# Project-MONAI/MONAI

Hardware: AMD Instinct MI355X
Metric: voxels/s sliding-window 3D seg (512^3 vol, 96^3 win, ov 0.5) at 1/8 GPU (higher is better)
Workload: dtype f32; 1 GPU; BasicUNet 5-class seed 1, 512^3 CT phantom in HBM, 96^3 win ov 0.5 gaussian, sw_batch 4 (engine: <= 64 windows per launch); parallelism=1 GPU

## Files before the change

### monai_amd/csrc/kernels/conv3d_wino_h2.h

```cpp
#pragma once
#include "common.h"
#include "conv3d_h2.h"

namespace mh {

constexpr int HWG_BY = 4, HWG_BX = 16;
constexpr int HWG_RY = HWG_BY + 2, HWG_RX = HWG_BX + 2;
constexpr int HWG_NP = HWG_RY * HWG_RX;
constexpr int HWG_PB = 144;
constexpr int HWG_DB = (HWG_NP + 1) * HWG_PB;
constexpr int HWG_ZB = 32 * 1024;
constexpr int HWG_OPS = 24;
constexpr int HWG_CIN = 32, HWG_CN = 32;
constexpr int HWG_WAVES = 8;
constexpr unsigned HWG_DROP = 0x80000000u;

__device__ __forceinline__ void hw_split4(const f32x4 v, u32x2& hi, u32x2& lo) {
    _Float16 h_[4], l_[4];
#pragma unroll
    for (int i = 0; i < 4; ++i) {
        h_[i] = (_Float16)v[i];
        float r = v[i] - (float)h_[i];
        MH_OPAQUE(r);
        l_[i] = (_Float16)r;
    }
    const f16x2 h01 = {h_[0], h_[1]}, h23 = {h_[2], h_[3]}, l01 = {l_[0], l_[1]}, l23 = {l_[2], l_[3]};
    hi = u32x2{__builtin_bit_cast(unsigned, h01), __builtin_bit_cast(unsigned, h23)};
    lo = u32x2{__builtin_bit_cast(unsigned, l01), __builtin_bit_cast(unsigned, l23)};
}

__device__ __forceinline__ f32x4 hw_fma4(const f32x4 a, const float s, const f32x4 c) { return __builtin_elementwise_fma(a, f32x4{s, s, s, s}, c); }
__device__ __forceinline__ void hw_split4p(const f32x4 v, const float m1, u32x2& hi, u32x2& lo) {
#ifdef MH_SIMT_EMULATOR
    f16x2 h01, l01, h23, l23;
    h2_split_pair(v[0], v[1], m1, h01, l01);
    h2_split_pair(v[2], v[3], m1, h23, l23);
    hi = u32x2{__builtin_bit_cast(unsigned, h01), __builtin_bit_cast(unsigned, h23)};
    lo = u32x2{__builtin_bit_cast(unsigned, l01), __builtin_bit_cast(unsigned, l23)};
#else
    unsigned h0, h1, l0, l1;
    asm("v_cvt_pk_f16_f32 %0, %1, %2" : "=v"(h0) : "v"(v[0]), "v"(v[1]));
    asm("v_cvt_pk_f16_f32 %0, %1, %2" : "=v"(h1) : "v"(v[2]), "v"(v[3]));
    asm("v_fma_mixlo_f16 %0, %1, %2, %3 op_sel_hi:[1,0,0]" : "=v"(l0) : "v"(h0), "v"(m1), "v"(v[0]));
    asm("v_fma_mixlo_f16 %0, %1, %2, %3 op_sel_hi:[1,0,0]" : "=v"(l1) : "v"(h1), "v"(m1), "v"(v[2]));
    asm("v_fma_mixhi_f16 %0, %1, %2, %3 op_sel:[1,0,0] op_sel_hi:[1,0,0]" : "+v"(l0) : "v"(h0), "v"(m1), "v"(v[1]));
    asm("v_fma_mixhi_f16 %0, %1, %2, %3 op_sel:[1,0,0] op_sel_hi:[1,0,0]" : "+v"(l1) : "v"(h1), "v"(m1), "v"(v[3]));
    hi = u32x2{h0, h1};
    lo = u32x2{l0, l1};
#endif
}
__device__ __forceinline__ float hw_xchg32(const float x, const int hi) {
#ifdef MH_SIMT_EMULATOR
    (void)hi;
    return __shfl_xor(x, 32);
#else
    const auto r = __builtin_amdgcn_permlane32_swap(__builtin_bit_cast(unsigned, x), __builtin_bit_cast(unsigned, x), false, false);
    return __builtin_bit_cast(float, hi ? r[0] : r[1]);
#endif
}
#ifdef MH_SIMT_EMULATOR
#define MH_HW_KEEP_BRANCH ((void)0)
#else
#define MH_HW_KEEP_BRANCH asm volatile("" ::: "memory")
#endif

template <bool STATS, bool ACC = false, bool POOL = false>
__global__ void __launch_bounds__(512)
conv3d_k3_h2w_kernel(Tensor in, const uint4* __restrict__ wp, const float* __restrict__ wtail, const float* __restrict__ bias, Tensor out,
                     float* __restrict__ stats, int bxn, int byn, int zchunk, unsigned nblk, float* __restrict__ pmax, float* __restrict__ pmin,
                     long long pool_n_stride) {
    __shared__ __attribute__((aligned(16))) char smem[3 * HWG_DB + 2 * HWG_ZB];
    __shared__ unsigned bound_s[4];
    char* const ds = smem;
    char* const zs_ = smem + 3 * HWG_DB;
    const int tid = threadIdx.x, lane = tid & 63;
    const int wave = __builtin_amdgcn_readfirstlane(tid >> 6);
    const int wi = wave & 3, jp = wave >> 2;
    const int Cout = out.C, D = out.D, H = out.H, W = out.W;
    const long long HW = (long long)H * W, DHW = (long long)D * HW;

    const unsigned ncg = (unsigned)(Cout / HWG_CN);
    unsigned lid = xcd_remap(blockIdx.x, gridDim.x);
    const int cg = (int)(lid % ncg);
    lid /= ncg;
    const unsigned b = lid % nblk;
    const int n = (int)(lid / nblk);
    const int x0 = (int)(b % bxn) * HWG_BX, y0 = (int)((b / bxn) % byn) * HWG_BY;
    const int zs = (int)(b / (bxn * byn)) * zchunk, ze = min(zs + zchunk, D);
    const int p_first = max(zs - 1, 0), p_last = min(ze, D - 1);

    unsigned soff;
    int loff[2];
    {
        const int pr = min(lane, 53);
        const int ly = pr / 9;
        int lx = 2 * (pr - 9 * ly);
        const int gy = y0 + ly - 1;
        int gx = x0 + lx - 1;
        if (gx < 0) { gx += 1; lx += 1; }
        if (gx + 1 >= W) { gx -= 1; lx -= 1; }
        const bool ok = lane < 54 && gy >= 0 && gy < H;
        soff = ok ? 4u * (unsigned)(gy * W + gx) : 0u;
        loff[0] = (ok ? ly * HWG_RX + lx : HWG_NP) * HWG_PB;
        loff[1] = (ok ? ly * HWG_RX + lx + 1 : HWG_NP) * HWG_PB;
    }
    for (int i = tid; i < (3 * HWG_DB + 2 * HWG_ZB) / 16; i += 512) reinterpret_cast<uint4*>(smem)[i] = make_uint4(0u, 0u, 0u, 0u);
    f32x4 nra, nrb, nrs;
    {
        unsigned mb = 0u;
        if (lane < HWG_CIN) {
            const float4 a = *reinterpret_cast<const float4*>(in.nrm + (long long)n * in.nrm_n_stride + 4LL * lane);
            const unsigned bb = abs_bits(a.w);
            mb = bb == 0u ? 0x7fc00000u : bb;
        }
        mb = wave_umax(mb);
        if (tid == 0) bound_s[0] = mb;
    }
    __syncthreads();
    int e_in = 0;
    bool poisoned = false;
    {
        const unsigned mb = bound_s[0];
        poisoned = mb >= 0x7f800000u;
        e_in = poisoned ? 0 : min(max(13 - ((int)(mb >> 23) - 126), -100), 100);
        const float p_ = __uint_as_float((unsigned)(e_in + 127) << 23);
#pragma unroll
        for (int i = 0; i < 4; ++i) {
            const float4 a = *reinterpret_cast<const float4*>(in.nrm + (long long)n * in.nrm_n_stride + 4LL * (4 * wave + i));
            nra[i] = a.x * p_; nrb[i] = a.y * p_; nrs[i] = a.z;
        }
    }
    f32x4 nrk;
#pragma unroll
    for (int i = 0; i < 4; ++i) nrk[i] = nrs[i] <= 1.0f ? __builtin_inff() : -__builtin_inff();
    const auto xrs = __builtin_amdgcn_make_buffer_rsrc(const_cast<float*>(in.data + (long long)n * in.n_stride + (long long)(4 * wave) * DHW), 0, 0x7fffffff, 0x00020000);
    const unsigned hw4 = (unsigned)(HW * 4);
    unsigned voff = soff + (unsigned)p_first * hw4;
    const unsigned cso1 = (unsigned)(DHW * 4), cso2 = 2u * cso1, cso3 = 3u * cso1;
    f32x2 xin[4];
#define MH_HW_LDX                                                                                     \
    {                                                                                                 \
        xin[0] = __builtin_bit_cast(f32x2, __builtin_amdgcn_raw_buffer_load_b64(xrs, voff, 0u, 0));   \
        xin[1] = __builtin_bit_cast(f32x2, __builtin_amdgcn_raw_buffer_load_b64(xrs, voff, cso1, 0)); \
        xin[2] = __builtin_bit_cast(f32x2, __builtin_amdgcn_raw_buffer_load_b64(xrs, voff, cso2, 0)); \
        xin[3] = __builtin_bit_cast(f32x2, __builtin_amdgcn_raw_buffer_load_b64(xrs, voff, cso3, 0)); \
    }
#define MH_HW_CONV(DBO)                                                                               \
    {                                                                                                 \
        char* const db_ = ds + (DBO) + 16 * wave;                                                     \
        _Pragma("unroll") for (int j = 0; j < 2; ++j) {                                               \
            f32x4 y_;                                                                                 \
            const f32x4 t_ = __builtin_elementwise_fma(f32x4{xin[0][j], xin[1][j], xin[2][j], xin[3][j]}, nra, nrb), u_ = t_ * nrs; \
            _Pragma("unroll") for (int i = 0; i < 4; ++i) y_[i] = __builtin_amdgcn_fmed3f(t_[i], u_[i], nrk[i]);       \
            *reinterpret_cast<f32x4*>(db_ + loff[j]) = y_;                                            \
        }                                                                                             \
    }
    int staged = p_first;
#define MH_HW_ADV { voff += staged < p_last ? hw4 : 0u; staged += 1; }

    u32x4 wu[HWG_OPS];
    {
        const u32x4* wg = reinterpret_cast<const u32x4*>(wp) + ((long long)(cg * 8 + wave) * HWG_OPS) * 64 + lane;
#pragma unroll
        for (int r = 0; r < HWG_OPS; ++r) wu[r] = wg[r * 64];
    }
#define MH_HW_U(SL, T, CB, PC) __builtin_bit_cast(f16x8, wu[(((SL) * 3 + (T)) * 2 + (CB)) * 2 + (PC)])

    const int rho = lane & 15, kg = lane >> 4;
    const int tty = (rho >= 4 && rho < 12) ? 1 : 0, ttx = rho < 4 ? rho : rho < 12 ? rho - 4 : rho - 8;
    const int ra = wi == 0 ? 0 : wi == 2 ? 2 : 1, rb = wi == 0 ? 2 : wi == 1 ? 2 : wi == 2 ? 1 : 3;
    const float sgn = wi == 1 ? 1.0f : -1.0f;
    const float fsg = jp ? -1.0f : 1.0f;
    const float m1 = h2_minus_one();
    const int ab0 = ((2 * tty + ra) * HWG_RX + 2 * ttx + jp) * HWG_PB + kg * 16;
    const int ab1 = ((2 * tty + rb) * HWG_RX + 2 * ttx + jp) * HWG_PB + kg * 16;

    f32x4 acc[3][2][2];
#pragma unroll
    for (int s = 0; s < 3; ++s)
#pragma unroll
        for (int j = 0; j < 2; ++j)
#pragma unroll
            for (int c = 0; c < 2; ++c) acc[s][j][c] = f32x4{0.0f, 0.0f, 0.0f, 0.0f};

    const int fcb = wave >> 2, frp = (wave >> 1) & 1, fh = wave & 1;
    const int il = 32 * fh + (lane & 31), fa = lane >> 5;
    const int g4 = il >> 4;
    const int fty = (g4 == 1 || g4 == 2) ? 1 : 0, ftx = (g4 >= 2 ? 4 : 0) + 2 * frp;
    const int co_l = fcb * 16 + (il & 15), co = cg * HWG_CN + co_l;
    const float bco = bias ? bias[co] : 0.0f;
    const float fs2 = fa ? -1.0f : 1.0f;
    const int zwr = wave * 4096 + lane * 16;
    const int zrd = fa * 4096 + fcb * 2048 + il * 16 + frp * 8;
    float inv_a, inv_b;
    {
        const int t_ = -((int)((__float_as_uint(wtail[1]) >> 23) & 0xffu) - 127) - e_in;
        const int t1_ = t_ / 2, t2_ = t_ - t1_;
        inv_a = poisoned ? __uint_as_float(0x7fc00000u) : __uint_as_float((unsigned)(t1_ + 127) << 23);
        inv_b = __uint_as_float((unsigned)(t2_ + 127) << 23);
    }
    const auto orsrc = __builtin_amdgcn_make_buffer_rsrc(out.data + (long long)n * out.n_stride + (long long)(cg * HWG_CN) * DHW, 0, (int)(HWG_CN * DHW * 4), 0x00020000);
    const unsigned ooff = 4u * (unsigned)((long long)co_l * DHW + (long long)(y0 + 2 * fty + fa) * W + x0 + 2 * ftx);
    float pivot = 0.0f;
    bool have_c = false;
    f32x4 s1 = {0.0f, 0.0f, 0.0f, 0.0f}, s2 = s1;
    const long long PHW = (long long)(H / 2) * (W / 2), PDHW = (long long)(D / 2) * PHW;
    const auto prs = __builtin_amdgcn_make_buffer_rsrc(POOL ? (fa ? pmin : pmax) + (long long)n * pool_n_stride + (long long)(cg * HWG_CN) * PDHW : out.data, 0, POOL ? (int)(HWG_CN * PDHW * 4) : 0, 0x00020000);
    const unsigned poff = 4u * (unsigned)((long long)co_l * PDHW + (long long)((y0 >> 1) + fty) * (W / 2) + (x0 >> 1) + ftx);
    const float pk_ = fa ? -__builtin_inff() : __builtin_inff();
    f32x2 hm = {0.0f, 0.0f};
    f32x4 pv = {0.0f, 0.0f, 0.0f, 0.0f};

    u32x4 ah[2], al[2];
#define MH_HW_XFORM(DBO)                                                                              \
    {                                                                                                 \
        const char* const db_ = ds + (DBO);                                                           \
        _Pragma("unroll") for (int h = 0; h < 2; ++h) {                                               \
            f32x4 r_[3];                                                                              \
            _Pragma("unroll") for (int bq = 0; bq < 3; ++bq) {                                        \
                const f32x4 u_ = *reinterpret_cast<const f32x4*>(db_ + ab0 + bq * HWG_PB + h * 64);   \
                const f32x4 v_ = *reinterpret_cast<const f32x4*>(db_ + ab1 + bq * HWG_PB + h * 64);   \
                r_[bq] = hw_fma4(v_, sgn, u_);                                                        \
            }                                                                                         \
            const f32x4 e_ = hw_fma4(r_[2], m1, r_[0]);                                               \
            f32x4 f_;                                                                                 \
            if (jp) { f_ = hw_fma4(r_[0], m1, r_[1]); MH_HW_KEEP_BRANCH; } else f_ = r_[1] + r_[2];   \
            u32x2 hh_, ll_;                                                                           \
            hw_split4p(e_, m1, hh_, ll_); ah[0][2 * h] = hh_[0]; ah[0][2 * h + 1] = hh_[1]; al[0][2 * h] = ll_[0]; al[0][2 * h + 1] = ll_[1]; \
            hw_split4p(f_, m1, hh_, ll_); ah[1][2 * h] = hh_[0]; ah[1][2 * h + 1] = hh_[1]; al[1][2 * h] = ll_[0]; al[1][2 * h + 1] = ll_[1]; \
        }                                                                                             \
    }
#define MH_HW_MM(S, SL, CB, A, B, FRESH)                                                              \
    acc[S][SL][CB] = __builtin_amdgcn_mfma_f32_16x16x32_f16(__builtin_bit_cast(f16x8, A), B, (FRESH) ? f32x4{0.0f, 0.0f, 0.0f, 0.0f} : acc[S][SL][CB], 0, 0, 0);
#define MH_HW_MMS(S0, S1, S2)                                                                         \
    _Pragma("unroll") for (int sl = 0; sl < 2; ++sl)                                                  \
        _Pragma("unroll") for (int cb = 0; cb < 2; ++cb) {                                            \
            MH_HW_MM(S0, sl, cb, ah[sl], MH_HW_U(sl, 0, cb, 0), true)  MH_HW_MM(S1, sl, cb, ah[sl], MH_HW_U(sl, 1, cb, 0), false) MH_HW_MM(S2, sl, cb, ah[sl], MH_HW_U(sl, 2, cb, 0), false) \
            MH_HW_MM(S0, sl, cb, al[sl], MH_HW_U(sl, 0, cb, 0), false) MH_HW_MM(S1, sl, cb, al[sl], MH_HW_U(sl, 1, cb, 0), false) MH_HW_MM(S2, sl, cb, al[sl], MH_HW_U(sl, 2, cb, 0), false) \
            MH_HW_MM(S0, sl, cb, ah[sl], MH_HW_U(sl, 0, cb, 1), false) MH_HW_MM(S1, sl, cb, ah[sl], MH_HW_U(sl, 1, cb, 1), false) MH_HW_MM(S2, sl, cb, ah[sl], MH_HW_U(sl, 2, cb, 1), false) \
        }
#define MH_HW_SKIP(S0)                                                                                \
    { _Pragma("unroll") for (int sl = 0; sl < 2; ++sl) _Pragma("unroll") for (int cb = 0; cb < 2; ++cb) acc[S0][sl][cb] = f32x4{0.0f, 0.0f, 0.0f, 0.0f}; }
#define MH_HW_ZOUT(S2, Q)                                                                             \
    {                                                                                                 \
        char* const zb_ = zs_ + ((Q) & 1) * HWG_ZB + zwr;                                             \
        _Pragma("unroll") for (int cb = 0; cb < 2; ++cb) {                                            \
            *reinterpret_cast<f32x4*>(zb_ + cb * 2048) = acc[S2][0][cb] + acc[S2][1][cb];             \
            *reinterpret_cast<f32x4*>(zb_ + cb * 2048 + 1024) = acc[S2][1][cb];                       \
        }                                                                                             \
    }
#define MH_HW_FINISH(Q, ON)                                                                           \
    {                                                                                                 \
        const bool on_ = (ON);                                                                        \
        const char* const zb_ = zs_ + ((Q) & 1) * HWG_ZB + zrd;                                       \
        f32x2 z0_[3], z1_[3];                                                                         \
        _Pragma("unroll") for (int i = 0; i < 3; ++i) {                                               \
            z0_[i] = *reinterpret_cast<const f32x2*>(zb_ + i * 4096) + *reinterpret_cast<const f32x2*>(zb_ + i * 4096 + 16384 + 1024);        \
            z1_[i] = *reinterpret_cast<const f32x2*>(zb_ + i * 4096 + 1024) - *reinterpret_cast<const f32x2*>(zb_ + i * 4096 + 16384);        \
        }                                                                                             \
        const f32x2 fs_ = {fs2, fs2};                                                                 \
        const f32x2 y0_ = __builtin_elementwise_fma(z0_[2], fs_, __builtin_elementwise_fma(z0_[1], fs_, z0_[0])) * inv_a; \
        const f32x2 y1_ = __builtin_elementwise_fma(z1_[2], fs_, __builtin_elementwise_fma(z1_[1], fs_, z1_[0])) * inv_a; \
        f32x4 o_ = {__builtin_fmaf(y0_[0], inv_b, bco), __builtin_fmaf(y1_[0], inv_b, bco), __builtin_fmaf(y0_[1], inv_b, bco), __builtin_fmaf(y1_[1], inv_b, bco)}; \
        if (ACC) o_ += pv;       \
        __builtin_amdgcn_raw_buffer_store_b128(__builtin_bit_cast(u32x4, o_), orsrc, on_ ? ooff + (unsigned)(Q) * (unsigned)(HW * 4) : HWG_DROP, 0, 0); \
        if (STATS) {         \
            pivot = (on_ && !have_c) ? o_[0] : pivot;                                                 \
            have_c = have_c || on_;                                                                   \
            const f32x4 d_ = o_ - pivot, dw_ = d_ * (on_ ? 1.0f : 0.0f);                              \
            s1 += dw_;                                                                                \
            s2 = __builtin_elementwise_fma(dw_, d_, s2);                                              \
        }                                                                                             \
        if (POOL && !(HWX_OFF & 32)) {          \
            const f32x2 mx_ = {fmaxf(o_[0], o_[1]), fmaxf(o_[2], o_[3])}, mn_ = {fminf(o_[0], o_[1]), fminf(o_[2], o_[3])}; \
            const f32x2 own_ = fa ? mn_ : mx_, snd_ = fa ? mx_ : mn_;                                 \
            const f32x2 rcv_ = {hw_xchg32(snd_[0], fa), hw_xchg32(snd_[1], fa)};                      \
            const f32x2 y_ = {__builtin_amdgcn_fmed3f(own_[0], rcv_[0], pk_), __builtin_amdgcn_fmed3f(own_[1], rcv_[1], pk_)};       \
            const f32x2 f_ = {__builtin_amdgcn_fmed3f(y_[0], hm[0], pk_), __builtin_amdgcn_fmed3f(y_[1], hm[1], pk_)}; \
            const unsigned po_ = (on_ && ((Q) & 1) && !(HWX_OFF & 64)) ? poff + (unsigned)((Q) >> 1) * (unsigned)(PHW * 4) : HWG_DROP; \
            __builtin_amdgcn_raw_buffer_store_b64(__builtin_bit_cast(u32x2, f_), prs, po_, 0, 0);     \
            hm = on_ ? y_ : hm;                                                                       \
        }                                                                                             \
    }
#ifdef HWX_PROF
#define MH_HW_T(K) { const long long t_ = __builtin_readcyclecounter(); tacc[K] += t_ - tlast; tlast = t_; }
    long long tacc[8] = {0, 0, 0, 0, 0, 0, 0, 0}, tlast = __builtin_readcyclecounter();
#else
#define MH_HW_T(K)
#endif
#ifndef HWX_OFF
#define HWX_OFF 0
#endif
#ifndef HWX_DEAL
#define HWX_DEAL 2
#endif
#define MH_HW_DEAL                                                                                    \
    if constexpr (ACC || POOL) {                                                                      \
        _Pragma("unroll") for (int g_ = 0; g_ < 36; ++g_) {                                           \
            __builtin_amdgcn_sched_group_barrier(0x008, 1, 0);                                        \
            __builtin_amdgcn_sched_group_barrier(0x100, 1, 0);                                        \
            __builtin_amdgcn_sched_group_barrier(0x006, HWX_DEAL, 0);                                 \
            __builtin_amdgcn_sched_group_barrier(0x230, 1, 0);                                        \
        }                                                                                             \
    }
#define MH_HW_ITER(P, R)                                                                              \
    {                                                                                                 \
        constexpr int S0 = (3 - (R)) % 3, S1 = (S0 + 1) % 3, S2 = (S0 + 2) % 3;       \
        constexpr int db0 = (R) * HWG_DB, db2 = (((R) + 2) % 3) * HWG_DB;             \
        const int p_ = (P);                                                                           \
        const bool valid_ = p_ >= p_first && p_ <= p_last;                                            \
        const int qf_ = p_ - 2;                                                                       \
        if (ACC) { const bool nx_ = qf_ >= zs && qf_ < ze; pv = __builtin_bit_cast(f32x4, __builtin_amdgcn_raw_buffer_load_b128(orsrc, nx_ ? ooff + (unsigned)qf_ * hw4 : HWG_DROP, 0, 0)); } \
        if (valid_) { if (!(HWX_OFF & 1)) MH_HW_XFORM(db0) }                                          \
        MH_HW_T(0)                                                                                    \
        __syncthreads();                                                                              \
        MH_HW_T(1)                                                                                    \
        if (valid_) {                                                                                 \
            __builtin_amdgcn_sched_barrier(0);                                                        \
            if (!(HWX_OFF & 2)) { MH_HW_CONV(db2) MH_HW_LDX MH_HW_ADV }                               \
            if (!(HWX_OFF & 4)) MH_HW_FINISH(qf_, qf_ >= zs && qf_ < ze)                              \
            if (!(HWX_OFF & 8)) MH_HW_MMS(S0, S1, S2)                                                 \
            MH_HW_DEAL                                                                                \
            __builtin_amdgcn_sched_barrier(0);                                                        \
        } else {                                                                                      \
            MH_HW_SKIP(S0)                                                                            \
            if (!(HWX_OFF & 4)) MH_HW_FINISH(qf_, qf_ >= zs && qf_ < ze)                              \
        }                                                                                             \
        if (!(HWX_OFF & 16)) if (p_ - 1 >= zs && p_ - 1 < ze) MH_HW_ZOUT(S2, p_ - 1)                  \
        MH_HW_T(2)                                                                                    \
        __syncthreads();                                                                              \
        MH_HW_T(3)                                                                                    \
    }

    {
        const int k0 = p_first - (zs - 1);
        MH_HW_LDX MH_HW_ADV
        __syncthreads();
        MH_HW_CONV((k0 % 3) * HWG_DB)
        MH_HW_LDX MH_HW_ADV
        MH_HW_CONV(((k0 + 1) % 3) * HWG_DB)
        MH_HW_LDX MH_HW_ADV
        __syncthreads();
    }
    if (jp) __syncthreads();
    for (int p = zs - 1; p <= ze + 1; p += 3) {
        MH_HW_ITER(p, 0)
        MH_HW_ITER(p + 1, 1)
        MH_HW_ITER(p + 2, 2)
    }
    if (!jp) __syncthreads();
#ifdef HWX_PROF
    if (blockIdx.x == 0 && lane == 0) { _Pragma("unroll") for (int k = 0; k < 8; ++k) reinterpret_cast<long long*>(pmax)[wave * 8 + k] = tacc[k]; }
#endif
#undef MH_HW_T
#undef MH_HW_DEAL
#undef MH_HW_ITER
#undef MH_HW_FINISH
#undef MH_HW_ZOUT
#undef MH_HW_SKIP
#undef MH_HW_MMS
#undef MH_HW_MM
#undef MH_HW_XFORM
#undef MH_HW_U
#undef MH_HW_ADV
#undef MH_HW_CONV
#undef MH_HW_LDX

    if (STATS) {
        Stat run;
        {
            const float a1 = (s1[0] + s1[1]) + (s1[2] + s1[3]), a2 = (s2[0] + s2[1]) + (s2[2] + s2[3]);
            run.n = 4.0f * (float)(ze - zs);
            const float dm = a1 / run.n;
            run.mean = pivot + dm;
            run.m2 = fmaxf(a2 - a1 * dm, 0.0f);
        }
#pragma unroll
        for (int o = 16; o <= 32; o <<= 1) {
            Stat ot;
            ot.n = __shfl_xor(run.n, o); ot.mean = __shfl_xor(run.mean, o); ot.m2 = __shfl_xor(run.m2, o);
            run = (lane & o) == 0 ? stat_merge(run, ot) : stat_merge(ot, run);
        }
        __syncthreads();
        float* red = reinterpret_cast<float*>(smem);
        if (lane < 16) { red[(wave * 16 + lane) * 3] = run.n; red[(wave * 16 + lane) * 3 + 1] = run.mean; red[(wave * 16 + lane) * 3 + 2] = run.m2; }
        __syncthreads();
        if (tid < HWG_CN) {
            const int cb = tid >> 4, c16 = tid & 15;
            Stat st;
            st.n = 0.0f; st.mean = 0.0f; st.m2 = 0.0f;
#pragma unroll
            for (int w = 0; w < 4; ++w) {
                Stat ot;
                ot.n = red[((4 * cb + w) * 16 + c16) * 3]; ot.mean = red[((4 * cb + w) * 16 + c16) * 3 + 1]; ot.m2 = red[((4 * cb + w) * 16 + c16) * 3 + 2];
                st = stat_merge(st, ot);
            }
            float* rec = stats + (((long long)n * Cout + cg * HWG_CN + tid) * nblk + b) * 3;
            rec[0] = st.n; rec[1] = st.mean; rec[2] = st.m2;
        }
    }
}

__global__ void conv3d_k3_h2w_scale_fix_kernel(float* __restrict__ tail) {
    if (threadIdx.x == 0 && blockIdx.x == 0) { tail[0] *= 4.0f; tail[1] *= 0.25f; }
}
__global__ void __launch_bounds__(256)
conv3d_k3_h2w_pack_kernel(const float* __restrict__ w, int Cin, int Cout, _Float16* __restrict__ packed, const float* __restrict__ tail) {
    const int idx = blockIdx.x * 256 + threadIdx.x;
    if (idx >= Cin * Cout) return;
    const int ci = idx % Cin, co = idx / Cin;
    const float s = tail[1];
    const double G[4][3] = {{1.0, 0.0, 0.0}, {0.5, 0.5, 0.5}, {0.5, -0.5, 0.5}, {0.0, 0.0, 1.0}};
    const int cg = co / HWG_CN, cb = (co % HWG_CN) / 16, nn = co % 16;
    const int kg = ci < 16 ? ci / 4 : (ci - 16) / 4, e = ci < 16 ? ci % 4 : 4 + (ci - 16) % 4;
    const int ln = kg * 16 + nn;
    for (int t = 0; t < 3; ++t) {
        double g[3][3], tm[4][3];
        for (int ky = 0; ky < 3; ++ky)
            for (int kx = 0; kx < 3; ++kx) g[ky][kx] = (double)w[((long long)co * Cin + ci) * 27 + t * 9 + ky * 3 + kx];
        for (int i = 0; i < 4; ++i)
            for (int kx = 0; kx < 3; ++kx) tm[i][kx] = G[i][0] * g[0][kx] + G[i][1] * g[1][kx] + G[i][2] * g[2][kx];
        for (int i = 0; i < 4; ++i)
            for (int j = 0; j < 4; ++j) {
                const double u = tm[i][0] * G[j][0] + tm[i][1] * G[j][1] + tm[i][2] * G[j][2];
                _Float16 pc[2];
                h2_split((float)(u * (double)s), pc[0], pc[1]);
                const int jpq = j >> 1, slot = (j == 0 || j == 3) ? 0 : 1;
                for (int p = 0; p < 2; ++p) {
                    const long long r = (((long long)(cg * 8 + jpq * 4 + i) * HWG_OPS) + ((slot * 3 + t) * 2 + cb) * 2 + p) * 64 + ln;
                    packed[r * 8 + e] = pc[p];
                }
            }
    }
}

}
```

Before: 206.4 million voxels/s.

## Split Winograd conv z-loop into steady-state and boundary iterations with uniform scalars

Restructures the main z-plane loop of the Winograd conv kernel into prologue and epilogue iterations plus a steady-state loop where validity checks are compile-time true, with the rotating accumulator and buffer slots unrolled by three. It also turns per-wave constants into SGPR values via readfirstlane, removes the jp branch in the input transform by negating the j==3 weights at pack time, replaces per-iteration output and pool address multiplies with running offsets, and splits the pool store into separate max and min descriptors. The aim is fewer VALU and branch instructions and less divergence in the hot loop. The cost is larger code and a changed weight-packing convention that must stay consistent with the kernel.

```diff
diff --git a/monai_amd/csrc/kernels/conv3d_wino_h2.h b/monai_amd/csrc/kernels/conv3d_wino_h2.h
--- a/monai_amd/csrc/kernels/conv3d_wino_h2.h
+++ b/monai_amd/csrc/kernels/conv3d_wino_h2.h
@@ -58,11 +58,8 @@
     return __builtin_bit_cast(float, hi ? r[0] : r[1]);
 #endif
 }
-#ifdef MH_SIMT_EMULATOR
-#define MH_HW_KEEP_BRANCH ((void)0)
-#else
-#define MH_HW_KEEP_BRANCH asm volatile("" ::: "memory")
-#endif
+
+__device__ __forceinline__ float hw_uniform(const float x) { return __builtin_bit_cast(float, __builtin_amdgcn_readfirstlane(__builtin_bit_cast(int, x))); }
 
 template <bool STATS, bool ACC = false, bool POOL = false>
 __global__ void __launch_bounds__(512)
@@ -127,12 +124,12 @@
 #pragma unroll
         for (int i = 0; i < 4; ++i) {
             const float4 a = *reinterpret_cast<const float4*>(in.nrm + (long long)n * in.nrm_n_stride + 4LL * (4 * wave + i));
-            nra[i] = a.x * p_; nrb[i] = a.y * p_; nrs[i] = a.z;
+            nra[i] = hw_uniform(a.x * p_); nrb[i] = a.y * p_; nrs[i] = a.z;
         }
     }
     f32x4 nrk;
 #pragma unroll
-    for (int i = 0; i < 4; ++i) nrk[i] = nrs[i] <= 1.0f ? __builtin_inff() : -__builtin_inff();
+    for (int i = 0; i < 4; ++i) nrk[i] = hw_uniform(nrs[i] <= 1.0f ? __builtin_inff() : -__builtin_inff());
     const auto xrs = __builtin_amdgcn_make_buffer_rsrc(const_cast<float*>(in.data + (long long)n * in.n_stride + (long long)(4 * wave) * DHW), 0, 0x7fffffff, 0x00020000);
     const unsigned hw4 = (unsigned)(HW * 4);
     unsigned voff = soff + (unsigned)p_first * hw4;
@@ -155,8 +152,7 @@
             *reinterpret_cast<f32x4*>(db_ + loff[j]) = y_;                                            \
         }                                                                                             \
     }
-    int staged = p_first;
-#define MH_HW_ADV { voff += staged < p_last ? hw4 : 0u; staged += 1; }
+#define MH_HW_ADV(S, F) { voff += ((F) || (S) < p_last) ? hw4 : 0u; }
 
     u32x4 wu[HWG_OPS];
     {
@@ -169,11 +165,12 @@
     const int rho = lane & 15, kg = lane >> 4;
     const int tty = (rho >= 4 && rho < 12) ? 1 : 0, ttx = rho < 4 ? rho : rho < 12 ? rho - 4 : rho - 8;
     const int ra = wi == 0 ? 0 : wi == 2 ? 2 : 1, rb = wi == 0 ? 2 : wi == 1 ? 2 : wi == 2 ? 1 : 3;
-    const float sgn = wi == 1 ? 1.0f : -1.0f;
-    const float fsg = jp ? -1.0f : 1.0f;
+    const float sgn = hw_uniform(wi == 1 ? 1.0f : -1.0f);
+    const float fsg = hw_uniform(jp ? -1.0f : 1.0f);
     const float m1 = h2_minus_one();
-    const int ab0 = ((2 * tty + ra) * HWG_RX + 2 * ttx + jp) * HWG_PB + kg * 16;
-    const int ab1 = ((2 * tty + rb) * HWG_RX + 2 * ttx + jp) * HWG_PB + kg * 16;
+    const int abm0 = ((2 * tty + ra) * HWG_RX + 2 * ttx + jp + 1) * HWG_PB + kg * 16;
+    const int abm1 = ((2 * tty + rb) * HWG_RX + 2 * ttx + jp + 1) * HWG_PB + kg * 16;
+    const int cst = jp ? -HWG_PB : HWG_PB;
 
     f32x4 acc[3][2][2];
 #pragma unroll
@@ -196,8 +193,8 @@
     {
         const int t_ = -((int)((__float_as_uint(wtail[1]) >> 23) & 0xffu) - 127) - e_in;
         const int t1_ = t_ / 2, t2_ = t_ - t1_;
-        inv_a = poisoned ? __uint_as_float(0x7fc00000u) : __uint_as_float((unsigned)(t1_ + 127) << 23);
-        inv_b = __uint_as_float((unsigned)(t2_ + 127) << 23);
+        inv_a = hw_uniform(poisoned ? __uint_as_float(0x7fc00000u) : __uint_as_float((unsigned)(t1_ + 127) << 23));
+        inv_b = hw_uniform(__uint_as_float((unsigned)(t2_ + 127) << 23));
     }
     const auto orsrc = __builtin_amdgcn_make_buffer_rsrc(out.data + (long long)n * out.n_stride + (long long)(cg * HWG_CN) * DHW, 0, (int)(HWG_CN * DHW * 4), 0x00020000);
     const unsigned ooff = 4u * (unsigned)((long long)co_l * DHW + (long long)(y0 + 2 * fty + fa) * W + x0 + 2 * ftx);
@@ -205,9 +202,12 @@
     bool have_c = false;
     f32x4 s1 = {0.0f, 0.0f, 0.0f, 0.0f}, s2 = s1;
     const long long PHW = (long long)(H / 2) * (W / 2), PDHW = (long long)(D / 2) * PHW;
-    const auto prs = __builtin_amdgcn_make_buffer_rsrc(POOL ? (fa ? pmin : pmax) + (long long)n * pool_n_stride + (long long)(cg * HWG_CN) * PDHW : out.data, 0, POOL ? (int)(HWG_CN * PDHW * 4) : 0, 0x00020000);
+    const auto prs_mx = __builtin_amdgcn_make_buffer_rsrc(POOL ? pmax + (long long)n * pool_n_stride + (long long)(cg * HWG_CN) * PDHW : out.data, 0, POOL ? (int)(HWG_CN * PDHW * 4) : 0, 0x00020000);
+    const auto prs_mn = __builtin_amdgcn_make_buffer_rsrc(POOL ? pmin + (long long)n * pool_n_stride + (long long)(cg * HWG_CN) * PDHW : out.data, 0, POOL ? (int)(HWG_CN * PDHW * 4) : 0, 0x00020000);
     const unsigned poff = 4u * (unsigned)((long long)co_l * PDHW + (long long)((y0 >> 1) + fty) * (W / 2) + (x0 >> 1) + ftx);
     const float pk_ = fa ? -__builtin_inff() : __builtin_inff();
+    unsigned oq = ooff + (unsigned)(zs - 3) * (unsigned)(HW * 4);
+    unsigned pq = poff + (unsigned)((zs - 3) >> 1) * (unsigned)(PHW * 4);
     f32x2 hm = {0.0f, 0.0f};
     f32x4 pv = {0.0f, 0.0f, 0.0f, 0.0f};
 
@@ -218,13 +218,12 @@
         _Pragma("unroll") for (int h = 0; h < 2; ++h) {                                               \
             f32x4 r_[3];                                                                              \
             _Pragma("unroll") for (int bq = 0; bq < 3; ++bq) {                                        \
-                const f32x4 u_ = *reinterpret_cast<const f32x4*>(db_ + ab0 + bq * HWG_PB + h * 64);   \
-                const f32x4 v_ = *reinterpret_cast<const f32x4*>(db_ + ab1 + bq * HWG_PB + h * 64);   \
+                const f32x4 u_ = *reinterpret_cast<const f32x4*>(db_ + abm0 + (bq - 1) * cst + h * 64); \
+                const f32x4 v_ = *reinterpret_cast<const f32x4*>(db_ + abm1 + (bq - 1) * cst + h * 64); \
                 r_[bq] = hw_fma4(v_, sgn, u_);                                                        \
             }                                                                                         \
-            const f32x4 e_ = hw_fma4(r_[2], m1, r_[0]);                                               \
-            f32x4 f_;                                                                                 \
-            if (jp) { f_ = hw_fma4(r_[0], m1, r_[1]); MH_HW_KEEP_BRANCH; } else f_ = r_[1] + r_[2];   \
+            const f32x4 e_ = r_[0] - r_[2];                                                           \
+            const f32x4 f_ = hw_fma4(r_[2], fsg, r_[1]);                                              \
             u32x2 hh_, ll_;                                                                           \
             hw_split4p(e_, m1, hh_, ll_); ah[0][2 * h] = hh_[0]; ah[0][2 * h + 1] = hh_[1]; al[0][2 * h] = ll_[0]; al[0][2 * h + 1] = ll_[1]; \
             hw_split4p(f_, m1, hh_, ll_); ah[1][2 * h] = hh_[0]; ah[1][2 * h + 1] = hh_[1]; al[1][2 * h] = ll_[0]; al[1][2 * h + 1] = ll_[1]; \
@@ -263,7 +262,7 @@
         const f32x2 y1_ = __builtin_elementwise_fma(z1_[2], fs_, __builtin_elementwise_fma(z1_[1], fs_, z1_[0])) * inv_a; \
         f32x4 o_ = {__builtin_fmaf(y0_[0], inv_b, bco), __builtin_fmaf(y1_[0], inv_b, bco), __builtin_fmaf(y0_[1], inv_b, bco), __builtin_fmaf(y1_[1], inv_b, bco)}; \
         if (ACC) o_ += pv;       \
-        __builtin_amdgcn_raw_buffer_store_b128(__builtin_bit_cast(u32x4, o_), orsrc, on_ ? ooff + (unsigned)(Q) * (unsigned)(HW * 4) : HWG_DROP, 0, 0); \
+        __builtin_amdgcn_raw_buffer_store_b128(__builtin_bit_cast(u32x4, o_), orsrc, on_ ? oq : HWG_DROP, 0, 0); \
         if (STATS) {         \
             pivot = (on_ && !have_c) ? o_[0] : pivot;                                                 \
             have_c = have_c || on_;                                                                   \
@@ -277,8 +276,9 @@
             const f32x2 rcv_ = {hw_xchg32(snd_[0], fa), hw_xchg32(snd_[1], fa)};                      \
             const f32x2 y_ = {__builtin_amdgcn_fmed3f(own_[0], rcv_[0], pk_), __builtin_amdgcn_fmed3f(own_[1], rcv_[1], pk_)};       \
             const f32x2 f_ = {__builtin_amdgcn_fmed3f(y_[0], hm[0], pk_), __builtin_amdgcn_fmed3f(y_[1], hm[1], pk_)}; \
-            const unsigned po_ = (on_ && ((Q) & 1) && !(HWX_OFF & 64)) ? poff + (unsigned)((Q) >> 1) * (unsigned)(PHW * 4) : HWG_DROP; \
-            __builtin_amdgcn_raw_buffer_store_b64(__builtin_bit_cast(u32x2, f_), prs, po_, 0, 0);     \
+            const unsigned po_ = (on_ && ((Q) & 1) && !(HWX_OFF & 64)) ? pq : HWG_DROP;               \
+            __builtin_amdgcn_raw_buffer_store_b64(__builtin_bit_cast(u32x2, f_), prs_mx, fa ? HWG_DROP : po_, 0, 0); \
+            __builtin_amdgcn_raw_buffer_store_b64(__builtin_bit_cast(u32x2, f_), prs_mn, fa ? po_ : HWG_DROP, 0, 0); \
             hm = on_ ? y_ : hm;                                                                       \
         }                                                                                             \
     }
@@ -295,7 +295,7 @@
 #define HWX_DEAL 2
 #endif
 #define MH_HW_DEAL                                                                                    \
-    if constexpr (ACC || POOL) {                                                                      \
+    {                                                                                                 \
         _Pragma("unroll") for (int g_ = 0; g_ < 36; ++g_) {                                           \
             __builtin_amdgcn_sched_group_barrier(0x008, 1, 0);                                        \
             __builtin_amdgcn_sched_group_barrier(0x100, 1, 0);                                        \
@@ -303,57 +303,67 @@
             __builtin_amdgcn_sched_group_barrier(0x230, 1, 0);                                        \
         }                                                                                             \
     }
-#define MH_HW_ITER(P, R)                                                                              \
-    {                                                                                                 \
-        constexpr int S0 = (3 - (R)) % 3, S1 = (S0 + 1) % 3, S2 = (S0 + 2) % 3;       \
-        constexpr int db0 = (R) * HWG_DB, db2 = (((R) + 2) % 3) * HWG_DB;             \
+#define MH_HW_ITER(P, S0, S1, S2, DB0, DB2, STEADY)                                                   \
+    {                                                                                                 \
         const int p_ = (P);                                                                           \
-        const bool valid_ = p_ >= p_first && p_ <= p_last;                                            \
+        const bool valid_ = (STEADY) || (p_ >= p_first && p_ <= p_last);                              \
         const int qf_ = p_ - 2;                                                                       \
-        if (ACC) { const bool nx_ = qf_ >= zs && qf_ < ze; pv = __builtin_bit_cast(f32x4, __builtin_amdgcn_raw_buffer_load_b128(orsrc, nx_ ? ooff + (unsigned)qf_ * hw4 : HWG_DROP, 0, 0)); } \
-        if (valid_) { if (!(HWX_OFF & 1)) MH_HW_XFORM(db0) }                                          \
+        const bool on_q_ = (STEADY) || (qf_ >= zs && qf_ < ze);                                       \
+        if (ACC) pv = __builtin_bit_cast(f32x4, __builtin_amdgcn_raw_buffer_load_b128(orsrc, on_q_ ? oq : HWG_DROP, 0, 0)); \
+        if (valid_) { if (!(HWX_OFF & 1)) MH_HW_XFORM(DB0) }                                          \
         MH_HW_T(0)                                                                                    \
         __syncthreads();                                                                              \
         MH_HW_T(1)                                                                                    \
+        if (!(STEADY) && !(HWX_OFF & 4)) MH_HW_FINISH(qf_, on_q_)                                     \
         if (valid_) {                                                                                 \
             __builtin_amdgcn_sched_barrier(0);                                                        \
-            if (!(HWX_OFF & 2)) { MH_HW_CONV(db2) MH_HW_LDX MH_HW_ADV }                               \
-            if (!(HWX_OFF & 4)) MH_HW_FINISH(qf_, qf_ >= zs && qf_ < ze)                              \
+            if (!(HWX_OFF & 2)) { MH_HW_CONV(DB2) MH_HW_LDX MH_HW_ADV(p_ + 3, STEADY) }               \
+            if ((STEADY) && !(HWX_OFF & 4)) MH_HW_FINISH(qf_, on_q_)                                  \
             if (!(HWX_OFF & 8)) MH_HW_MMS(S0, S1, S2)                                                 \
-            MH_HW_DEAL                                                                                \
+            if constexpr ((STEADY) && (ACC || POOL)) MH_HW_DEAL                                       \
             __builtin_amdgcn_sched_barrier(0);                                                        \
-        } else {                                                                                      \
-            MH_HW_SKIP(S0)                                                                            \
-            if (!(HWX_OFF & 4)) MH_HW_FINISH(qf_, qf_ >= zs && qf_ < ze)                              \
-        }                                                                                             \
-        if (!(HWX_OFF & 16)) if (p_ - 1 >= zs && p_ - 1 < ze) MH_HW_ZOUT(S2, p_ - 1)                  \
+        } else MH_HW_SKIP(S0)                                                                         \
+        if (!(HWX_OFF & 16)) if ((STEADY) || (p_ - 1 >= zs && p_ - 1 < ze)) MH_HW_ZOUT(S2, p_ - 1)    \
+        oq += hw4;                                                                                    \
+        if (POOL) pq += (qf_ & 1) ? (unsigned)(PHW * 4) : 0u;                                         \
         MH_HW_T(2)                                                                                    \
         __syncthreads();                                                                              \
         MH_HW_T(3)                                                                                    \
     }
+#define MH_HW_ITER_ENDS(P)                                                                            \
+    {                                                                                                 \
+        const int db0_ = kb * HWG_DB, db2_ = (kb == 0 ? 2 : kb - 1) * HWG_DB;                         \
+        MH_HW_ITER(P, 0, 1, 2, db0_, db2_, false)                                                     \
+        _Pragma("unroll") for (int sl = 0; sl < 2; ++sl) _Pragma("unroll") for (int cb = 0; cb < 2; ++cb) { acc[2][sl][cb] = acc[1][sl][cb]; acc[1][sl][cb] = acc[0][sl][cb]; } \
+        kb = kb == 2 ? 0 : kb + 1;                                                                    \
+    }
 
     {
         const int k0 = p_first - (zs - 1);
-        MH_HW_LDX MH_HW_ADV
+        MH_HW_LDX MH_HW_ADV(p_first, false)
         __syncthreads();
         MH_HW_CONV((k0 % 3) * HWG_DB)
-        MH_HW_LDX MH_HW_ADV
+        MH_HW_LDX MH_HW_ADV(p_first + 1, false)
         MH_HW_CONV(((k0 + 1) % 3) * HWG_DB)
-        MH_HW_LDX MH_HW_ADV
+        MH_HW_LDX MH_HW_ADV(p_first + 2, false)
         __syncthreads();
     }
     if (jp) __syncthreads();
-    for (int p = zs - 1; p <= ze + 1; p += 3) {
-        MH_HW_ITER(p, 0)
-        MH_HW_ITER(p + 1, 1)
-        MH_HW_ITER(p + 2, 2)
-    }
+    int p = zs - 1, kb = 0;
+    for (; p <= zs + 1; ++p) MH_HW_ITER_ENDS(p)
+    for (const int p_steady = min(ze - 2, p_last - 6); p <= p_steady; p += 3) {
+        MH_HW_ITER(p, 0, 1, 2, 0, 2 * HWG_DB, true)
+        MH_HW_ITER(p + 1, 2, 0, 1, HWG_DB, 0, true)
+        MH_HW_ITER(p + 2, 1, 2, 0, 2 * HWG_DB, HWG_DB, true)
+    }
+    for (; p <= ze + 1; ++p) MH_HW_ITER_ENDS(p)
     if (!jp) __syncthreads();
 #ifdef HWX_PROF
     if (blockIdx.x == 0 && lane == 0) { _Pragma("unroll") for (int k = 0; k < 8; ++k) reinterpret_cast<long long*>(pmax)[wave * 8 + k] = tacc[k]; }
 #endif
 #undef MH_HW_T
 #undef MH_HW_DEAL
+#undef MH_HW_ITER_ENDS
 #undef MH_HW_ITER
 #undef MH_HW_FINISH
 #undef MH_HW_ZOUT
@@ -428,7 +438,7 @@
                 const int jpq = j >> 1, slot = (j == 0 || j == 3) ? 0 : 1;
                 for (int p = 0; p < 2; ++p) {
                     const long long r = (((long long)(cg * 8 + jpq * 4 + i) * HWG_OPS) + ((slot * 3 + t) * 2 + cb) * 2 + p) * 64 + ln;
-                    packed[r * 8 + e] = pc[p];
+                    packed[r * 8 + e] = j == 3 ? -pc[p] : pc[p];
                 }
             }
     }
```

After: 207.4 million voxels/s (median of 6 runs). No clear change (+0.5%).
